# brendisurfs/Distributed-Backtesting-Exploration

Measured on AMD Instinct MI355X. Metric: bar-evals/sec (symbols x params x bars), higher is better.
Workload: dtype f64+int64; 1 GPU; BASELINE config 2: SMA fast/slow crossover, 5,000 symbols x 2,520 daily bars x 400 params per GPU; symbols_total=5000, symbols_per_gpu=5000, bars=2520, params=400, topk=100, parallelism=dp1 (contiguous symbol shards; exchange: none)

## Files before the change

### distributed-backtesting-exploration_amd/csrc/device_common.h

```cpp
#pragma once
#include <type_traits>

#include "internal.h"

namespace bt {

__host__ __device__ inline uint64_t trade_mix(uint64_t w) {
    const uint64_t z = (w ^ (w >> 29)) * 0xBF58476D1CE4E5B9ULL;
    return z ^ (z >> 32);
}
__host__ __device__ inline uint64_t trade_mix_et(uint32_t e, uint32_t t, bool lg) {
    const uint32_t lo = e ^ (t << 2) ^ (t << 31);
    const uint32_t hi = (t >> 1) ^ (lg ? 0x40000002u : 0u);
    const uint64_t z = (((uint64_t)hi << 32) | lo) * 0xBF58476D1CE4E5B9ULL;
    return z ^ (z >> 32);
}
constexpr int kDstLevels = 6;
constexpr int kKeyStride = kTile + 1;

typedef __int128 i128;
typedef __attribute__((address_space(3))) double lds_f64;

struct __attribute__((aligned(16))) Agg {
    int32_t mx, mn, dd, du;
};

__device__ __forceinline__ Agg agg_one(int32_t x) { return Agg{x, x, 0, 0}; }

__device__ __forceinline__ Agg agg_sel(bool c, const Agg& a, const Agg& b) {
    return Agg{c ? a.mx : b.mx, c ? a.mn : b.mn, c ? a.dd : b.dd, c ? a.du : b.du};
}

__device__ __forceinline__ Agg agg_merge(const Agg& a, const Agg& b) {
    Agg r;
    r.mx = max(a.mx, b.mx);
    r.mn = min(a.mn, b.mn);
    r.dd = max(max(a.dd, b.dd), a.mx - b.mn);
    r.du = max(max(a.du, b.du), b.mx - a.mn);
    return r;
}

__device__ __forceinline__ int dst_row(int a, int b) {
    return __builtin_clz((unsigned)(a ^ b) | 1u) - (32 - kDstLevels);
}
__device__ __forceinline__ const Agg* dst_rowp(const Agg* D, int a, int b) {
    return D - (32 - kDstLevels) * kTile + __builtin_clz((unsigned)(a ^ b) | 1u) * kTile;
}

__device__ __forceinline__ Agg dst_query(const Agg* D, const int32_t* cT, int a, int b) {
    if (a == b) return agg_one(cT[a]);
    const int r = dst_row(a, b);
    return agg_merge(D[r * kTile + a], D[r * kTile + b]);
}

__device__ __forceinline__ Agg dst_query_bf(const Agg* D, int a, int b) {
    const Agg* Dr = dst_rowp(D, a, b);
    return agg_merge(Dr[a], Dr[b]);
}

__device__ __forceinline__ Agg dst_query_w(const Agg* D, int a, int b) {
    const Agg* Dr = dst_rowp(D, a, b);
    const int4 u = *reinterpret_cast<const int4*>(Dr + a);
    const int4 v = *reinterpret_cast<const int4*>(Dr + b);
    asm volatile("" ::"v"(u.x), "v"(u.y), "v"(u.z), "v"(u.w), "v"(v.x), "v"(v.y), "v"(v.z), "v"(v.w));
    return agg_merge(Agg{u.x, u.y, u.z, u.w}, Agg{v.x, v.y, v.z, v.w});
}

__host__ __device__ inline double key_recip(int W) { return (1.0 / (double)W) * (1.0 + 0x1p-47); }

constexpr Agg kAggId = {0, 0x7FFFFFFF, 0, 0};

__device__ __forceinline__ int64_t wave_iscan_i64(int64_t x) {
    uint32_t lo = (uint32_t)x, hi = (uint32_t)((uint64_t)x >> 32);
#define BT_DPP_STEP(ctrl, rmask)                                                      \
    {                                                                                 \
        const uint32_t ylo = __builtin_amdgcn_update_dpp(0u, lo, ctrl, rmask, 0xf, false); \
        const uint32_t yhi = __builtin_amdgcn_update_dpp(0u, hi, ctrl, rmask, 0xf, false); \
        const uint64_t r = (((uint64_t)hi << 32) | lo) + (((uint64_t)yhi << 32) | ylo);   \
        lo = (uint32_t)r;                                                             \
        hi = (uint32_t)(r >> 32);                                                     \
    }
    BT_DPP_STEP(0x111, 0xf)
    BT_DPP_STEP(0x112, 0xf)
    BT_DPP_STEP(0x114, 0xf)
    BT_DPP_STEP(0x118, 0xf)
    BT_DPP_STEP(0x142, 0xa)
    BT_DPP_STEP(0x143, 0xc)
#undef BT_DPP_STEP
    return (int64_t)(((uint64_t)hi << 32) | lo);
}

#define BT_S64_CTRLS(X)                                                                   \
    X("row_shr:1 row_mask:0xf bank_mask:0xf bound_ctrl:1")                                \
    X("row_shr:2 row_mask:0xf bank_mask:0xf bound_ctrl:1")                                \
    X("row_shr:4 row_mask:0xf bank_mask:0xf bound_ctrl:1")                                \
    X("row_shr:8 row_mask:0xf bank_mask:0xf bound_ctrl:1")                                \
    X("row_bcast:15 row_mask:0xa bank_mask:0xf")                                          \
    X("row_bcast:31 row_mask:0xc bank_mask:0xf")
__device__ __forceinline__ int64_t wave_iscan_i64_ac(int64_t x) {
    uint32_t lo = (uint32_t)x, hi = (uint32_t)((uint64_t)x >> 32);
#define BT_S64_ONE(ctrl)                                                                   \
    "s_nop 1\n"                                                                            \
    "v_add_co_u32_dpp %0, vcc, %0, %0 " ctrl "\n"                                          \
    "v_addc_co_u32_dpp %1, vcc, %1, %1, vcc " ctrl "\n"
    asm volatile(BT_S64_CTRLS(BT_S64_ONE) "s_nop 1" : "+v"(lo), "+v"(hi) : : "vcc");
#undef BT_S64_ONE
    return (int64_t)(((uint64_t)hi << 32) | lo);
}
__device__ __forceinline__ void wave_iscan2_i64_ac(int64_t& x, int64_t& y) {
    uint32_t xl = (uint32_t)x, xh = (uint32_t)((uint64_t)x >> 32);
    uint32_t yl = (uint32_t)y, yh = (uint32_t)((uint64_t)y >> 32);
#define BT_S64_TWO(ctrl)                                                                   \
    "v_add_co_u32_dpp %0, vcc, %0, %0 " ctrl "\n"                                          \
    "v_addc_co_u32_dpp %1, vcc, %1, %1, vcc " ctrl "\n"                                    \
    "v_add_co_u32_dpp %2, vcc, %2, %2 " ctrl "\n"                                          \
    "v_addc_co_u32_dpp %3, vcc, %3, %3, vcc " ctrl "\n"
    asm volatile("s_nop 1\n" BT_S64_CTRLS(BT_S64_TWO) "s_nop 1"
                 : "+v"(xl), "+v"(xh), "+v"(yl), "+v"(yh) : : "vcc");
#undef BT_S64_TWO
    x = (int64_t)(((uint64_t)xh << 32) | xl);
    y = (int64_t)(((uint64_t)yh << 32) | yl);
// ... 98 lines not shown
```

### distributed-backtesting-exploration_amd/csrc/engine.cpp

```cpp
#include <hip/hip_runtime.h>

#include <algorithm>
#include <atomic>
#include <charconv>
#include <chrono>
#include <cmath>
#include <cstdio>
#include <cstdlib>
#include <cstring>
#include <exception>
#include <string>
#include <thread>
#include <unordered_map>
#include <vector>

#include "csv.h"
#include "internal.h"

using namespace bt;

namespace {

thread_local std::string g_err;

void set_err(const std::string& s) { g_err = s; }

struct HipFail {
    std::string msg;
};

#define HIPCHK(x)                                                                              \
    do {                                                                                       \
        hipError_t e_ = (x);                                                                   \
        if (e_ != hipSuccess)                                                                  \
            throw HipFail{std::string(#x) + ": " + hipGetErrorString(e_)};                     \
    } while (0)

template <class T>
struct DevBuf {
    T* p = nullptr;
    size_t n = 0;
    void ensure(size_t want) {
        if (want <= n && p) return;
        if (p) (void)hipFree(p);
        p = nullptr;
        n = 0;
        if (want == 0) return;
        HIPCHK(hipMalloc(&p, want * sizeof(T)));
        n = want;
    }
    void release() {
        if (p) (void)hipFree(p);
        p = nullptr;
        n = 0;
    }
};

uint32_t next_pow2(uint32_t x) {
    uint32_t r = 1;
    while (r < x) r <<= 1;
    return r;
}

}

void bt::set_last_error(const std::string& s) { set_err(s); }

constexpr int64_t kNtrRing = 64;

struct bt_engine {
    bt_config cfg{};
    std::vector<int32_t> ax[4];
    Grid grid{};
    int32_t P = 0;
    hipStream_t stream = nullptr;
    bool own_stream = false;
    DevBuf<int32_t> d_axes[4];
    std::vector<SymDesc> syms;
    int64_t rows = 0;
    DevBuf<SymDesc> d_syms;
    DevBuf<int32_t> d_c, d_h, d_l;
    DevBuf<bt_summary> d_sum[2];
    DevBuf<uint64_t> d_key[2];
    DevBuf<unsigned long long> d_ntr_ring;
    unsigned long long* ntr[2] = {nullptr, nullptr};
    int cur = 0;
    int64_t nrun = 0;
    DevBuf<bt_sums> d_sums;
    DevBuf<bt_trade> d_trades;
    int32_t seg_req = 0, seg_burn = kDefaultBurnTiles, seg_last = 1;
    bool seg_burn_set = false;
    DevBuf<SegRec> d_seg;
    DevBuf<double> d_segema;
    DevBuf<unsigned long long> d_refixed;
    DevBuf<unsigned long long> d_dbg;
    hipStream_t tstream = nullptr;
    hipEvent_t ev_kdone = nullptr;
    hipEvent_t ev_tdone[2] = {nullptr, nullptr};
    bool tdone_armed[2] = {false, false};
    DevBuf<unsigned int> d_hist, d_counts;
    DevBuf<unsigned long long> d_state, d_above, d_cand;
    DevBuf<bt_topk_rec> d_top;
    bt_topk_rec* h_top = nullptr;
    bt_topk_rec* h_slot[BT_PIPE_SLOTS] = {};
    hipEvent_t slot_ev[BT_PIPE_SLOTS] = {};
    bool slot_armed[BT_PIPE_SLOTS] = {};
    bool topk_ready = false;
    bool ran = false;
    std::vector<std::pair<hipEvent_t, hipEvent_t>> ev_pending, ev_pool;
    double kernel_ms = 0.0;
    int64_t launches = 0;
    int32_t* h_stage[3] = {nullptr, nullptr, nullptr};
    size_t stage_rows[3] = {0, 0, 0};
    bt_summary* h_sum = nullptr;
    size_t h_sum_n = 0;
    hipEvent_t ev_batch[4] = {nullptr, nullptr, nullptr, nullptr};
    bt_batch_profile prof{};
    int64_t n_errors = 0;
    DevBuf<uint8_t> d_replay;
};

namespace {

void activate(bt_engine* e) { HIPCHK(hipSetDevice(e->cfg.device)); }

bool has_hl(const bt_engine* e) { return e->cfg.strategy == BT_BOLL; }

const char* kernel_name(int32_t strategy) {
    switch (strategy) {
        case BT_SMA_CROSS: return "bt::sma_kernel";
// ... 39 lines not shown
            e->grid.nc = e->grid.nd = 1;
            e->grid.band_bps = c.band_bps;
            e->grid.wmax = *std::max_element(e->ax[1].begin(), e->ax[1].end());
            e->grid.ring = (e->grid.wmax + 5 * kTile - 1) / kTile * kTile;
            if (ema_lds_bytes(e->grid, 1) > 160 * 1024) return "EMA grid needs more LDS than a CU has (OLS windows too long)";
            break;
        }
        case BT_BOLL: {
            if (!(err = copy_axis(0, c.bwin, c.n_bwin, "bwin", 1, 1 << 16)).empty()) return err;
            if (!(err = copy_axis(1, c.k_num, c.n_k, "k_num", 0, 1 << 20)).empty()) return err;
            if (!(err = copy_axis(2, c.sl_bps, c.n_sl, "sl_bps", 0, 9999)).empty()) return err;
            if (!(err = copy_axis(3, c.tp_bps, c.n_tp, "tp_bps", 0, 9999)).empty()) return err;
            if (c.k_den < 1 || c.k_den > (1 << 20)) return "k_den out of range";
            e->grid.na = c.n_bwin;
            e->grid.nb = c.n_k;
            e->grid.nc = c.n_sl;
            e->grid.nd = c.n_tp;
            e->grid.k_den = c.k_den;
            e->grid.wmax = *std::max_element(e->ax[0].begin(), e->ax[0].end());
            const int64_t kmax = std::max<int64_t>(c.k_den, *std::max_element(e->ax[1].begin(), e->ax[1].end()));
            if ((int64_t)e->grid.wmax * kmax >= (1LL << 32)) return "Bollinger grid outside the exact int128 range (window * k >= 2^32)";
            e->grid.ring = (e->grid.wmax + 4 * kTile - 1) / kTile * kTile;
            for (int q = 0; q < 8; ++q) {
                const int64_t kn = q < c.n_k ? e->ax[1][q] : 0;
                e->grid.kn2[q] = (double)(kn * kn);
            }
            e->grid.kmin_idx = (int32_t)(std::min_element(e->ax[1].begin(), e->ax[1].end()) - e->ax[1].begin());
            if (boll_lds_bytes(e->grid) > 160 * 1024) return "Bollinger grid needs more LDS than a CU has (windows too long)";
            break;
        }
        default:
            return "unknown strategy";
    }
    const int64_t P = (int64_t)e->grid.na * e->grid.nb * e->grid.nc * e->grid.nd;
    if (P <= 0 || P > (1 << 20)) return "parameter grid too large";
    e->P = (int32_t)P;
    e->grid.n_params = e->P;
    if (c.annualization <= 0) return "annualization must be positive";
    e->grid.sqrt_ann = std::sqrt((double)c.annualization);
    if (c.topk < 0 || c.topk > kTopkMax) return "topk must be in [0, 1024]";
    if ((c.flags & BT_FLAG_PARITY) && c.trade_cap <= 0) return "parity mode needs trade_cap > 0";
    return "";
}

void upload_grid(bt_engine* e) {
    const int32_t** dst[4] = {&e->grid.a, &e->grid.b, &e->grid.c, &e->grid.d};
    for (int i = 0; i < 4; ++i) {
        *dst[i] = nullptr;
        if (e->ax[i].empty()) continue;
        e->d_axes[i].ensure(e->ax[i].size());
        HIPCHK(hipMemcpy(e->d_axes[i].p, e->ax[i].data(), e->ax[i].size() * 4, hipMemcpyHostToDevice));
        *dst[i] = e->d_axes[i].p;
    }
}

int64_t align_rows(int64_t bars) { return (bars + kRowAlign - 1) / kRowAlign * kRowAlign; }

void sync_all(bt_engine* e);

void set_dataset(bt_engine* e, std::vector<SymDesc>&& syms, int64_t rows) {
    sync_all(e);
    e->syms = std::move(syms);
    e->rows = rows;
    const size_t n_sym = e->syms.size();
    e->d_syms.ensure(std::max<size_t>(1, n_sym));
    if (n_sym)
        HIPCHK(hipMemcpyAsync(e->d_syms.p, e->syms.data(), n_sym * sizeof(SymDesc),
                              hipMemcpyHostToDevice, e->stream));
    const size_t r = std::max<int64_t>(1, rows);
    e->d_c.ensure(r);
    if (has_hl(e)) {
        e->d_h.ensure(r);
        e->d_l.ensure(r);
    }
    e->ran = false;
}

void layout(bt_engine* e, int32_t n_sym, const int32_t* bars, const int64_t* ids) {
    std::vector<SymDesc> syms((size_t)n_sym);
    int64_t off = 0;
    for (int32_t s = 0; s < n_sym; ++s) {
        syms[s].off = off;
        syms[s].bars = bars[s];
        syms[s].id = (int32_t)ids[s];
        off += align_rows(bars[s]);
    }
    set_dataset(e, std::move(syms), off);
}

template <class T>
void ensure_pinned(T*& p, size_t& have, size_t want) {
    if (want <= have && p) return;
    if (p) HIPCHK(hipHostFree(p));
    p = nullptr;
    have = 0;
    HIPCHK(hipHostMalloc(&p, std::max<size_t>(want, 1) * sizeof(T)));
    have = std::max<size_t>(want, 1);
}

TopkWork topk_work(bt_engine* e) {
    return TopkWork{e->d_hist.p, e->d_state.p, e->d_counts.p, e->d_above.p, e->d_cand.p,
                    kTopkCap, e->d_top.p + 1, reinterpret_cast<int32_t*>(e->d_top.p)};
}

void sync_all(bt_engine* e) {
    HIPCHK(hipStreamSynchronize(e->stream));
// ... 540 lines not shown
        e = new bt_engine();
        e->cfg = *cfg;
        std::string m = validate_and_copy(e, *cfg);
        if (!m.empty()) {
            delete e;
            return fail(m);
        }
        e->cfg.fast = e->cfg.slow = e->cfg.span = e->cfg.ols = nullptr;
        e->cfg.bwin = e->cfg.k_num = e->cfg.sl_bps = e->cfg.tp_bps = nullptr;
        int ndev = 0;
        HIPCHK(hipGetDeviceCount(&ndev));
        if (cfg->device < 0 || cfg->device >= ndev)
            throw HipFail{"HIP device " + std::to_string(cfg->device) + " not present (" +
                          std::to_string(ndev) + " visible)"};
        activate(e);
        if (cfg->stream) {
            e->stream = (hipStream_t)cfg->stream;
        } else {
            HIPCHK(hipStreamCreateWithFlags(&e->stream, hipStreamNonBlocking));
            e->own_stream = true;
        }
        HIPCHK(hipStreamCreateWithFlags(&e->tstream, hipStreamNonBlocking));
        HIPCHK(hipEventCreateWithFlags(&e->ev_kdone, hipEventDisableTiming));
        for (int b = 0; b < 2; ++b) HIPCHK(hipEventCreateWithFlags(&e->ev_tdone[b], hipEventDisableTiming));
        upload_grid(e);
#ifdef BT_PROFILING
        if (const char* ab = getenv("BT_ABLATE")) e->grid.ablate = atoi(ab);
#endif
        return e;
    } catch (const HipFail& f) {
        delete e;
        return fail(f.msg);
    } catch (const std::exception& x) {
        delete e;
        return fail(std::string("exception: ") + x.what());
    }
}

void bt_engine_destroy(bt_engine* e) {
    if (!e) return;
    try {
        (void)hipSetDevice(e->cfg.device);
        if (e->stream) (void)hipStreamSynchronize(e->stream);
        if (e->tstream) (void)hipStreamSynchronize(e->tstream);
        for (auto& ev : e->ev_pending) {
            (void)hipEventDestroy(ev.first);
            (void)hipEventDestroy(ev.second);
        }
        for (auto& ev : e->ev_pool) {
            (void)hipEventDestroy(ev.first);
            (void)hipEventDestroy(ev.second);
        }
        for (auto& b : e->d_axes) b.release();
        e->d_syms.release();
        e->d_c.release();
        e->d_h.release();
        e->d_l.release();
        for (int b = 0; b < 2; ++b) {
            e->d_sum[b].release();
            e->d_key[b].release();
            if (e->ev_tdone[b]) (void)hipEventDestroy(e->ev_tdone[b]);
            e->ev_tdone[b] = nullptr;
            e->tdone_armed[b] = false;
        }
        if (e->ev_kdone) (void)hipEventDestroy(e->ev_kdone);
        e->ev_kdone = nullptr;
        e->d_ntr_ring.release();
        e->d_sums.release();
        e->d_trades.release();
        e->d_seg.release();
        e->d_segema.release();
        e->d_refixed.release();
        e->d_dbg.release();
        e->d_replay.release();
        e->d_hist.release();
        e->d_counts.release();
        e->d_state.release();
        e->d_above.release();
        e->d_cand.release();
        e->d_top.release();
        if (e->h_top) (void)hipHostFree(e->h_top);
        e->h_top = nullptr;
        for (int i = 0; i < BT_PIPE_SLOTS; ++i) {
            if (e->h_slot[i]) (void)hipHostFree(e->h_slot[i]);
            if (e->slot_ev[i]) (void)hipEventDestroy(e->slot_ev[i]);
            e->h_slot[i] = nullptr;
            e->slot_ev[i] = nullptr;
            e->slot_armed[i] = false;
        }
        e->topk_ready = false;
        for (int i = 0; i < 3; ++i)
            if (e->h_stage[i]) (void)hipHostFree(e->h_stage[i]);
        if (e->h_sum) (void)hipHostFree(e->h_sum);
        for (hipEvent_t& ev : e->ev_batch)
            if (ev) (void)hipEventDestroy(ev);
        if (e->own_stream && e->stream) (void)hipStreamDestroy(e->stream);
        if (e->tstream) (void)hipStreamDestroy(e->tstream);
        e->tstream = nullptr;
    } catch (...) {
    }
    delete e;
}

int32_t bt_num_params(const bt_engine* e) { return e ? e->P : -1; }

int32_t bt_set_segments(bt_engine* e, int32_t segments, int32_t burn_tiles) {
// ... 350 lines not shown
```

### distributed-backtesting-exploration_amd/csrc/internal.h

```cpp
#pragma once
#include <hip/hip_runtime.h>
#include <stdint.h>

#include <string>

#include "../../include/bt.h"

#ifdef BT_PROFILING
#define BT_ABL(g, bit) (((g).ablate & (bit)) != 0)
#define BT_PRIO(g, shift, dflt) (BT_ABL(g, 1 << 20) ? (((g).ablate >> (shift)) & 3) : (dflt))
#else
#define BT_ABL(g, bit) false
#define BT_PRIO(g, shift, dflt) (dflt)
#endif
constexpr int kDbgSlots = 80, kDbgBlocks = 1024;

namespace bt {

constexpr int kTile = 64;
constexpr int kRowAlign = 64;

struct SymDesc {
    int64_t off;
    int32_t bars;
    int32_t id;
};

struct Grid {
    int32_t strategy;
    int32_t n_params;
    int32_t na, nb, nc, nd;
    int32_t band_bps, k_den;
    int32_t wmax;
    int32_t ring;
    double sqrt_ann;
    double kn2[8];
    int32_t kmin_idx;
    int32_t ablate;
    const int32_t* a;
    const int32_t* b;
    const int32_t* c;
    const int32_t* d;
};

struct Out {
    bt_summary* sum;
    uint64_t* key;
    bt_sums* sums;
    bt_trade* trades;
    int32_t trade_cap;
    unsigned long long* n_trades;
    unsigned long long* dbg;
};

struct SegRec {
    int32_t ntr, expo;
    int32_t start_pos, start_e;
    int32_t end_pos, end_e, end_ce, pad;
    int32_t end_agg[4];
    int64_t R;
    int64_t A, B, C, D;
    uint64_t h;
    uint64_t s1lo;
    int64_t s1hi;
    uint64_t s2lo;
    int64_t s2hi;
};
static_assert(sizeof(SegRec) == 128, "SegRec layout");
struct SmaSegRec {
    int32_t ntr;
    int32_t e0;
    int32_t start_pos, end_pos;
    int32_t end_e, end_ce;
    int32_t x1, px1;
    int32_t agg1[4];
    int32_t end_agg[4];
    int64_t R;
    int64_t B, C, D;
    uint64_t h;
    uint64_t s1lo, s2lo;
    int32_t s1hi, s2hi;
};
static_assert(sizeof(SmaSegRec) == sizeof(SegRec), "SmaSegRec is one 128-B SegRec slot");
struct SegArgs {
    SegRec* rec;
    int8_t* pos;
    unsigned long long* refixed;
    double* ema;
    int32_t G;
    int32_t burn_tiles;
};
constexpr int kDefaultBurnTiles = 64;
constexpr int kEmaSegStride = 128;
hipError_t launch_gen(const SymDesc* syms, int32_t n_sym, uint64_t seed, int32_t freq,
                      int32_t* o, int32_t* h, int32_t* l, int32_t* c, hipStream_t st);
size_t sma_lds_bytes(const Grid& g);
// ... 14 lines not shown
size_t boll_lds_bytes(const Grid& g);
hipError_t launch_ema_ols(const SymDesc* syms, int32_t n_sym, const int32_t* close, const Grid& g,
                          const Out& out, bool parity, const SegArgs& seg, hipStream_t st);
int32_t ema_auto_segments(int32_t n_sym, int32_t n_params, int32_t max_bars, int32_t burn_tiles);
int32_t ema_burn_tiles(int32_t max_span);
hipError_t launch_boll(const SymDesc* syms, int32_t n_sym, const int32_t* high, const int32_t* low,
                       const int32_t* close, const Grid& g, const Out& out, bool parity,
                       const SegArgs& seg, hipStream_t st);
int32_t boll_auto_segments(int32_t n_sym, int32_t n_params, int32_t max_bars);

struct ReplayLane {
    int64_t off;
    int32_t bars;
    int32_t param;
};
struct ReplayOut {
    bt_summary* sum;
    bt_trade* trades;
    int32_t trade_cap;
    int64_t* equity;
    int8_t* pos;
    int64_t pitch;
};
hipError_t launch_replay(const ReplayLane* lanes, int32_t n, const int32_t* high, const int32_t* low,
                         const int32_t* close, const Grid& g, const ReplayOut& o, hipStream_t st);

constexpr int kTopkCap = 2048;
constexpr int kTopkMax = 1024;
struct TopkWork {
    unsigned int* hist;
    unsigned long long* state;
    unsigned int* counts;
    unsigned long long* above;
    unsigned long long* cand;
    int cap;
    bt_topk_rec* out;
    int32_t* out_n;
};
hipError_t launch_topk(const uint64_t* key, const bt_summary* sum, const SymDesc* syms,
                       int64_t n, int32_t P, int32_t k, const TopkWork& w, hipStream_t st, bool lds_free_hist = false);
hipError_t launch_topk_init(const TopkWork& w, hipStream_t st);

void set_last_error(const std::string& s);
inline bool topk_less(const bt_topk_rec& a, const bt_topk_rec& b);
struct ExchangeView {
    hipStream_t tstream;
    int32_t device, topk;
    const bt_topk_rec* d_top;
    const unsigned long long* d_ntr;
    int64_t bar_evals;
};
bool engine_exchange_view(bt_engine* e, ExchangeView& v, std::string& err);
void engine_exchange_enqueued(bt_engine* e);

__host__ __device__ inline uint64_t order_key(double x) {
    union { double d; uint64_t u; } v;
    v.d = x;
    return (v.u >> 63) ? ~v.u : (v.u | 0x8000000000000000ULL);
}

__host__ __device__ inline double i128_to_double(uint64_t lo, int64_t hi) {
    const bool neg = hi < 0;
    uint64_t mh = (uint64_t)hi, ml = lo;
    if (neg) {
        ml = ~ml + 1;
        mh = ~mh + (ml == 0 ? 1 : 0);
    }
    if (mh == 0 && ml == 0) return 0.0;
    int lz = mh ? __builtin_clzll(mh) : 64 + __builtin_clzll(ml);
    uint64_t nh, nl;
    if (lz >= 64) {
        nh = ml << (lz - 64);
        nl = 0;
    } else if (lz == 0) {
        nh = mh;
        nl = ml;
    } else {
        nh = (mh << lz) | (ml >> (64 - lz));
        nl = ml << lz;
    }
    uint64_t mant = nh >> 11;
    const uint64_t rem_hi = nh & 0x7FFULL;
    const uint64_t half = 0x400ULL;
    bool up;
    if (rem_hi > half) up = true;
    else if (rem_hi < half) up = false;
    else up = (nl != 0) || (mant & 1);
    mant += up ? 1 : 0;
    double r = (double)mant;
#ifdef __HIP_DEVICE_COMPILE__
    r = ldexp(r, 75 - lz);
#else
    r = __builtin_ldexp(r, 75 - lz);
#endif
    return neg ? -r : r;
}

inline bool topk_less(const bt_topk_rec& a, const bt_topk_rec& b) {
    const uint64_t ka = order_key(a.sharpe), kb = order_key(b.sharpe);
    if (ka != kb) return ka > kb;
    if (a.sym != b.sym) return a.sym < b.sym;
    return a.param < b.param;
}

__host__ __device__ inline double sharpe_fx(uint64_t s1lo, int64_t s1hi, uint64_t s2lo,
                                            int64_t s2hi, int32_t bars, double sqrt_ann) {
// ... 10 lines not shown
```

### distributed-backtesting-exploration_amd/csrc/k_sma.hip

```cpp
#include <algorithm>
#include <cmath>
#include <cstdlib>

#include "tile_common.h"

namespace bt {

namespace {

constexpr int kKS = kTile + 4;
constexpr int kStages = 3;
constexpr int kDstStages = 2;
constexpr int kKeyGrab = 4;
constexpr int kCmpDepth1 = 2;

struct SmaLds {
    size_t ring, keys, invw, win, dst, ct, ql, nar, ctr, total;
};

__host__ __device__ inline SmaLds sma_lds_layout(int ring, int nw) {
    SmaLds L;
    size_t o = 0;
    auto take = [&](size_t bytes) { size_t r = o; o += (bytes + 15) & ~size_t(15); return r; };
    L.ring = take((size_t)ring * 8);
    const int nwp = (nw + kKeyGrab - 1) / kKeyGrab * kKeyGrab;
    L.keys = take((size_t)2 * nwp * kKS * 4);
    L.invw = take((size_t)nwp * 8);
    L.win = take((size_t)nwp * 4);
    L.dst = take((size_t)kDstStages * kDstLevels * kTile * sizeof(Agg));
    L.ct = take((size_t)kStages * kTile * 4);
    L.ql = take((size_t)kStages * 2 * kTile * 8);
    L.nar = take((size_t)kStages * 4);
    L.ctr = take(4);
    L.total = o;
    return L;
}

struct ScanCarry {
    int64_t P;
    int32_t prevc;
    uint32_t tv;
};

__device__ __forceinline__ int32_t load_close(const int32_t* __restrict__ crow, int B, int t) {
    return t < B ? crow[t] : 0;
}

__device__ __forceinline__ void stage_ring(int32_t c, int B, int t0, int lane, int R, double* ring,
                                           int32_t* cT, int64_t* ql, int32_t* narrow,
                                           ScanCarry& cy) {
    const int t = t0 + lane;
    const bool valid = t < B;
    const int32_t cp = (int32_t)__builtin_amdgcn_update_dpp((uint32_t)cy.prevc, (uint32_t)c,
                                                            0x138, 0xf, 0xf, false);
    const int64_t inc = wave_iscan_i64((int64_t)c);
    ring[(t + 1) & (R - 1)] = (double)(cy.P + inc);
    cT[lane] = c;
    int64_t q = 0, q2 = 0;
    uint32_t dv = 0;
    if (valid && t >= 1) {
        fixed_ret(c, cp, q, q2);
        dv = (uint32_t)abs(c - cp);
    }
    ql[lane] = wave_iscan_i64(q);
    ql[kTile + lane] = wave_iscan_i64(q2);
    const bool big = __ballot(dv >= (1u << 25)) != 0;
    const uint32_t tvt = __builtin_amdgcn_readlane(wave_iscan_u32(min(dv, 1u << 25)), 63);
    cy.tv = big ? (1u << 31) : min(cy.tv + tvt, 1u << 31);
    if (lane == 0) *narrow = cy.tv < (1u << 30);
    cy.P += lane63_i64(inc);
    cy.prevc = (int32_t)__builtin_amdgcn_readlane((uint32_t)c, 63);
}

__device__ __forceinline__ uint32_t grab_issue(uint32_t* ctr, int lane) {
    uint32_t v = 0;
    if (lane == 0) v = atomicAdd(ctr, (uint32_t)kKeyGrab);
    return v;
}

__device__ __forceinline__ int32_t floor_key(double F, double iw) {
    return (int32_t)(F * iw);
}

__host__ __device__ inline uint32_t key_round_len(int nwp, int nwaves) {
    return (uint32_t)kKeyGrab * ((uint32_t)nwp / kKeyGrab + 1 + (uint32_t)nwaves);
}

__device__ __forceinline__ void stage_keys(int t0, int B, int nw, int nwp, int nf, int wmax, int R,
                                           double* ring, const int32_t* win,
                                           const double* invw, int32_t* K, uint32_t* ctr,
                                           uint32_t round, int nwaves, int lane,
                                           const int32_t* cTr, Agg* Dr) {
    const int t = t0 + lane;
    const double top = ring[(t + 1) & (R - 1)];
    const bool full = t0 + 1 - wmax >= 0 && t0 + kTile <= B;
    const uint32_t base = round * key_round_len(nwp, nwaves);
    uint32_t w = __builtin_amdgcn_readlane(grab_issue(ctr, lane), 0) - base;
#pragma unroll 1
    while (w < (uint32_t)(nwp + kKeyGrab)) {
        const uint32_t vn = grab_issue(ctr, lane);
        if (w == 0) {
            dst_build<true>(cTr[lane], lane, Dr);
            w = __builtin_amdgcn_readlane(vn, 0) - base;
            continue;
        }
        w -= kKeyGrab;
        int Wv[kKeyGrab];
        double Iv[kKeyGrab], Fv[kKeyGrab];
#pragma unroll
        for (int q = 0; q < kKeyGrab; q += 4) {
            const int4 W4 = *reinterpret_cast<const int4*>(win + w + q);
            Wv[q] = W4.x; Wv[q + 1] = W4.y; Wv[q + 2] = W4.z; Wv[q + 3] = W4.w;
        }
#pragma unroll
        for (int q = 0; q < kKeyGrab; q += 2) {
            const double2 I2 = *reinterpret_cast<const double2*>(invw + w + q);
            Iv[q] = I2.x; Iv[q + 1] = I2.y;
        }
#pragma unroll
        for (int q = 0; q < kKeyGrab; ++q) {
            Wv[q] = __builtin_amdgcn_readfirstlane(Wv[q]);
            Fv[q] = top - ring[(t + 1 - Wv[q]) & (R - 1)];
        }
        int32_t* Kw = K + w * kKS + lane;
        if (full) {
#pragma unroll
            for (int q = 0; q < kKeyGrab; ++q) Kw[q * kKS] = floor_key(Fv[q], Iv[q]);
        } else {
            const bool tin = t < B;
#pragma unroll
            for (int q = 0; q < kKeyGrab; ++q) {
                const int32_t kq = floor_key(Fv[q], Iv[q]);
                Kw[q * kKS] = (tin && t + 1 - Wv[q] >= 0) ? kq : ((int)(w + q) < nf ? -1 : -2);
            }
        }
        w = __builtin_amdgcn_readlane(vn, 0) - base;
    }
}

__device__ __forceinline__ void cmp4(uint32_t& l, uint32_t& z, const int4& x, const int4& y) {
    const uint32_t d0 = (uint32_t)(x.x - y.x), d1 = (uint32_t)(x.y - y.y);
    const uint32_t d2 = (uint32_t)(x.z - y.z), d3 = (uint32_t)(x.w - y.w);
    l = __builtin_amdgcn_alignbit(l, d0, 31);
    l = __builtin_amdgcn_alignbit(l, d1, 31);
    l = __builtin_amdgcn_alignbit(l, d2, 31);
    l = __builtin_amdgcn_alignbit(l, d3, 31);
    z = min(min(z, d0), d1);
    z = min(min(z, d2), d3);
}

__device__ __forceinline__ uint64_t eq_word(const int32_t* k1, const int32_t* k2) {
    uint64_t e = 0;
#pragma unroll 1
    for (int b = 0; b < kTile; ++b) e |= (uint64_t)(k1[b] == k2[b]) << b;
    return e;
}

}

struct SmaAcct {
    int32_t pos, e, ce, sb, ntr, e0;
    int32_t g32, m32, r32;
    int64_t R, gap, mdd;
    uint64_t ps1, ps2, h;
    I96 s1, s2;
    Agg agg;
    int64_t Bq, C, D;
    int32_t carried, x1, px1;
    Agg agg1;
};


template <bool PARITY, bool MERGE = true, bool SEG = false, bool NARROW = false>
__device__ __forceinline__ void sma_close(SmaAcct& a, const Agg& seg, int t, int32_t cx,
                                          bt_trade* tr, int cap) {
    const Agg st = MERGE ? agg_merge(a.agg, seg) : seg;
    if (SEG && MERGE && a.carried) {
        a.x1 = t;
        a.px1 = cx;
        a.agg1 = st;
        a.carried = 0;
        a.ntr++;
        return;
    }
    const bool lg = a.pos > 0;
    const int32_t lo = lg ? st.mn - a.ce : a.ce - st.mx;
    const int32_t hi = lg ? st.mx - a.ce : a.ce - st.mn;
    const int32_t path = lg ? st.dd : st.du;
    const int32_t pnl = lg ? cx - a.ce : a.ce - cx;
// ... 55 lines not shown
                     "v"((uint32_t)(qb >> 32)));
        seg = agg_merge(d1, d2);
    } else {
        seg = dst_query_bf(D, a.sb, b);
        cx = cT[b];
        qb = (uint64_t)ql[b];
    }
    alt = qb - alt;
    sma_close<PARITY, FIRST, SEG, NARROW>(a, seg, t0 + b, cx, tr, cap);
    sma_open<FIRST>(a, b, t0 + b, cx, -a.pos);
}

template <bool PARITY, bool ONE_TRIP, bool SEG, bool NARROW>
__device__ __forceinline__ void sma_flips(SmaAcct& a, uint64_t F, int t0, int bl, uint64_t LONG,
                                          const int32_t* cT, const int64_t* ql, const Agg* D,
                                          bt_trade* tr, int cap) {
    const uint64_t FX = (bl >= 0 && bl < 64) ? (F & (1ULL << bl)) : 0ULL;
    F ^= FX;
    if (a.pos == 0 && F != 0) {
        const int b = __builtin_ctzll(F);
        F &= F - 1;
        const int np = ((LONG >> b) & 1) ? 1 : -1;
        const uint64_t qx = (uint64_t)ql[b];
        a.ps1 += np > 0 ? (uint64_t)0 - qx : qx;
        a.ps2 -= (uint64_t)ql[kTile + b];
        a.e0 = t0 + b;
        sma_open(a, b, t0 + b, cT[b], np);
    }
    uint64_t alt = 0;
    if (F) sma_reverse<PARITY, ONE_TRIP, true, SEG, NARROW>(a, F, alt, t0, cT, ql, D, tr, cap);
    while (F) sma_reverse<PARITY, ONE_TRIP, false, SEG, NARROW>(a, F, alt, t0, cT, ql, D, tr, cap);
    a.ps1 += a.pos > 0 ? (uint64_t)0 - (alt << 1) : alt << 1;
    if (FX) {
        const int b = bl;
        const uint64_t qx = (uint64_t)ql[b];
        sma_close<PARITY, true, SEG, NARROW>(a, dst_query_bf(D, a.sb, b), t0 + b, cT[b], tr, cap);
        a.ps1 += a.pos > 0 ? qx : (uint64_t)0 - qx;
        a.ps2 += (uint64_t)ql[kTile + b];
        a.pos = 0;
    }
}

template <bool PARITY, bool STAMPS, bool ONE_TRIP, bool SEG>
__device__ __forceinline__ void sma_body(const SymDesc* __restrict__ syms,
                                         const int32_t* __restrict__ close, const Grid& g,
                                         const Out& out, int dedicated, const SegArgs& sg,
                                         int fix_seg) {
    extern __shared__ __attribute__((aligned(16))) unsigned char smem[];
    const int nf = g.na, ns = g.nb, nw = nf + ns;
    const int R = g.ring;
    const SmaLds LL = sma_lds_layout(R, nw);
    double* ring = reinterpret_cast<double*>(smem + LL.ring);
    int32_t* keys = reinterpret_cast<int32_t*>(smem + LL.keys);
    double* invw = reinterpret_cast<double*>(smem + LL.invw);
    int32_t* win = reinterpret_cast<int32_t*>(smem + LL.win);
    Agg* dst = reinterpret_cast<Agg*>(smem + LL.dst);
    int32_t* cts = reinterpret_cast<int32_t*>(smem + LL.ct);
    int64_t* qls = reinterpret_cast<int64_t*>(smem + LL.ql);
    int32_t* nars = reinterpret_cast<int32_t*>(smem + LL.nar);
    uint32_t* ctr = reinterpret_cast<uint32_t*>(smem + LL.ctr);

    const int tid = threadIdx.x;
    const int lane = tid & 63;
    const int wave = __builtin_amdgcn_readfirstlane(tid >> 6);
    const int nwaves = (int)blockDim.x >> 6;
    const bool helper = (tid >> 6) == nwaves - 1;
    const int nparam_threads = dedicated ? (int)blockDim.x - 64 : (int)blockDim.x;
    const SymDesc sd = syms[blockIdx.x];
    const int B = sd.bars;
    const int ntiles = (B + kTile - 1) / kTile;
    const int P = g.n_params;
    const int j = blockIdx.y * nparam_threads + tid;
    const bool active = tid < nparam_threads && j < P;
    const int kf = active ? j % nf : 0;
    const int ks = nf + (active ? j / nf : 0);
    const int p = (kf * ns) + (ks - nf);
    const int32_t* crow = close + sd.off;

    SegRange sr{0, 0, 0, 0, ntiles};
    SmaSegRec* mine = nullptr;
    size_t ipos = 0, npos = 0;
    if (SEG) {
        sr = seg_range(sg, fix_seg, ntiles, g.wmax);
        const size_t per_seg = (size_t)gridDim.x * P;
        ipos = sr.seg * per_seg + (size_t)blockIdx.x * P + p;
        npos = (size_t)sg.G * per_seg;
        mine = reinterpret_cast<SmaSegRec*>(sg.rec) + ipos;
        if (fix_seg > 0) {
            if (!__syncthreads_or(active && sg.pos[ipos] != sg.pos[npos + ipos - per_seg])) return;
            if (tid == 0) atomicAdd(sg.refixed, 1ULL);
        }
    }
    const int T_scan = sr.T_scan, T_walk = sr.T_walk, T_acct = sr.T_acct, T_end = sr.T_end;

    const int nwp = (nw + kKeyGrab - 1) / kKeyGrab * kKeyGrab;
    const uint32_t key_round = key_round_len(nwp, nwaves);
    for (int w = tid; w < nwp; w += blockDim.x) {
        const int W = w < nf ? g.a[w] : (w < nw ? g.b[w - nf] : 1);
        win[w] = W;
        invw[w] = key_recip(W);
    }
    if (tid == 0) {
        ring[(T_scan * kTile) & (R - 1)] = 0.0;
        *ctr = (uint32_t)T_walk * key_round;
    }
    __syncthreads();
    const int warm = max(win[kf], win[ks]) - 1;
    const uint32_t fsw = (uint32_t)win[kf] | ((uint32_t)win[ks] << 16);

    ScanCarry cy{0, (T_scan > 0 && T_scan * kTile - 1 < B) ? crow[T_scan * kTile - 1] : 0};
    if (SEG && helper && T_scan < T_walk) {
        constexpr int kLookAhead = 8;
        int32_t cn[kLookAhead];
#pragma unroll
        for (int u = 0; u < kLookAhead; ++u) cn[u] = load_close(crow, B, (T_scan + u) * kTile + lane);
#pragma unroll 1
        for (int T0 = T_scan; T0 < T_walk; T0 += kLookAhead) {
#pragma unroll
            for (int u = 0; u < kLookAhead; ++u) {
                const int T = T0 + u;
                if (T < T_walk) {
                    const int32_t c = cn[u];
                    cn[u] = load_close(crow, B, (T + kLookAhead) * kTile + lane);
                    const int64_t inc = wave_iscan_i64((int64_t)c);
                    ring[(T * kTile + lane + 1) & (R - 1)] = (double)(cy.P + inc);
                    cy.P += lane63_i64(inc);
                    cy.prevc = (int32_t)__builtin_amdgcn_readlane((uint32_t)c, 63);
                }
            }
        }
    }
    int32_t cpre = 0;
    if (helper) {
        const int b0 = T_walk * kTile;
        const int32_t c0 = load_close(crow, B, b0 + lane), c1 = load_close(crow, B, b0 + kTile + lane);
        cpre = load_close(crow, B, b0 + 2 * kTile + lane);
        const int s0 = T_walk % kStages, s1 = (T_walk + 1) % kStages;
        if (T_walk < T_end) stage_ring(c0, B, b0, lane, R, ring, cts + s0 * kTile, qls + s0 * 2 * kTile, nars + s0, cy);
        __syncthreads();
        if (T_walk + 1 < T_end)
            stage_ring(c1, B, b0 + kTile, lane, R, ring, cts + s1 * kTile, qls + s1 * 2 * kTile, nars + s1, cy);
    } else {
        __syncthreads();
    }
    if (T_walk < T_end)
        stage_keys(T_walk * kTile, B, nw, nwp, nf, g.wmax, R, ring, win, invw,
                   keys + (T_walk & 1) * nwp * kKS, ctr, (uint32_t)T_walk, nwaves, lane,
                   cts + (T_walk % kStages) * kTile, dst + (T_walk % kDstStages) * kDstLevels * kTile);
    __syncthreads();

    SmaAcct a;
    a.pos = a.e = a.ce = a.sb = a.ntr = a.e0 = 0;
    a.g32 = a.m32 = a.r32 = 0;
    a.R = a.gap = a.mdd = 0;
    a.ps1 = a.ps2 = 0;
    a.h = 0;
    a.s1.clear();
    a.s2.clear();
    a.agg = kAggId;
    a.Bq = a.C = a.D = kNegInf;
    a.carried = a.x1 = a.px1 = 0;
    a.agg1 = kAggId;
    int32_t start_pos = 0;
    if (SEG && fix_seg > 0 && active) a.pos = sg.pos[npos + ipos - (size_t)gridDim.x * P];
    auto enter_acct = [&]() {
        start_pos = a.pos;
        a.carried = a.pos != 0;
        a.agg = kAggId;
        a.sb = 0;
        a.R = 0;
        a.Bq = a.C = a.D = kNegInf;
        a.ntr = 0;
        a.h = 0;
        a.s1.clear();
        a.s2.clear();
        a.ps1 = a.ps2 = 0;
        a.e0 = -1;
        a.x1 = -1;
        a.px1 = 0;
        a.agg1 = kAggId;
    };
    if (SEG && T_walk == T_acct) enter_acct();
    bt_trade* tr = nullptr;
    auto result_index = [&]() -> size_t {
        int le = lane;
        asm volatile("" : "+v"(le));
        const int je = blockIdx.y * nparam_threads + wave * 64 + le;
        return (size_t)blockIdx.x * P + (size_t)((je % nf) * ns + je / nf);
    };
    const size_t gi = (size_t)blockIdx.x * P + p;
    if (PARITY && active) tr = out.trades + gi * out.trade_cap;
    const int cap = out.trade_cap;

    constexpr bool stamps = STAMPS;
    uint64_t st_acc[7] = {0, 0, 0, 0, 0, 0, 0};
    uint64_t st_prev = 0;
#define BT_STAMP(i)                                             \
    if (stamps) {                                               \
        const uint64_t now_ = __builtin_amdgcn_s_memtime();     \
        st_acc[i] += now_ - st_prev;                            \
        st_prev = now_;                                         \
    }
    if (stamps) st_prev = __builtin_amdgcn_s_memtime();

    auto tile_step = [&](auto narrow_tag, const int k) __attribute__((always_inline)) {
        constexpr bool NARROW = decltype(narrow_tag)::value;
        const int t0 = k * kTile;
        if (helper && k + 2 < T_end && !BT_ABL(g, 1)) {
            if (!BT_ABL(g, 32)) __builtin_amdgcn_s_setprio(2);
            const int s = (k + 2) % kStages;
            stage_ring(cpre, B, t0 + 2 * kTile, lane, R, ring, cts + s * kTile,
                       qls + s * 2 * kTile, nars + s, cy);
            cpre = load_close(crow, B, t0 + 3 * kTile + lane);
            __builtin_amdgcn_s_setprio(0);
        }
        BT_STAMP(0)
        if (SEG && active && k == T_acct && k != T_walk) enter_acct();
        if (active) {
            if (ONE_TRIP) __builtin_amdgcn_s_setprio(1);
            const int s = k % kStages;
            const int32_t* cT = cts + s * kTile;
            const int64_t* ql = qls + s * 2 * kTile;
            const Agg* D = dst + (k % kDstStages) * kDstLevels * kTile;
            const int32_t* K = keys + (k & 1) * nwp * kKS;
            const int4* k1 = reinterpret_cast<const int4*>(K + kf * kKS);
            const int4* k2 = reinterpret_cast<const int4*>(K + ks * kKS);
            uint32_t l0 = 0, l1 = 0, z = ~0u;
            if (!BT_ABL(g, 4)) {
#pragma unroll
                for (int v = 0; v < 16; ++v) {
                    if (v < 8) cmp4(l0, z, k1[v], k2[v]);
                    else cmp4(l1, z, k1[v], k2[v]);
                    if (ONE_TRIP ? ((v % kCmpDepth1) == kCmpDepth1 - 1) : (v & 1))
                        __builtin_amdgcn_sched_barrier(0);
                }
            }
            BT_STAMP(2)
            uint64_t L = ((uint64_t)__builtin_bitreverse32(l1) << 32) | __builtin_bitreverse32(l0);
            const int lastdec = B - 2 - t0;
            const int wb = warm - t0;
            const int bl = B - 1 - t0;
            uint64_t LONG, F;
            if (z != 0 && wb <= 0 && lastdec >= 63) {
                LONG = ~L;
                F = (LONG ^ ((LONG << 1) | (uint64_t)(a.pos == 1))) | (uint64_t)(a.pos == 0);
            } else {
                uint64_t vm = lastdec >= 63 ? ~0ULL : (lastdec < 0 ? 0ULL : ((1ULL << (lastdec + 1)) - 1));
                vm &= wb <= 0 ? ~0ULL : (wb >= 64 ? 0ULL : (~0ULL << wb));
                uint64_t G, T = 0;
                if (z != 0) {
                    G = ~L & vm;
                } else {
                    const uint64_t E = eq_word(K + kf * kKS, K + ks * kKS);
                    G = ~(L | E) & vm;
                    T = E & vm;
                }
                L &= vm;
                while (T) {
                    const int b = __builtin_ctzll(T);
                    T &= T - 1;
                    const int t = t0 + b;
                    const double top = ring[(t + 1) & (R - 1)];
                    const int fw = (int)(fsw & 0xffffu), sw = (int)(fsw >> 16);
                    const int64_t Fs = (int64_t)(top - ring[(t + 1 - fw) & (R - 1)]) * sw;
                    const int64_t Lf = (int64_t)(top - ring[(t + 1 - sw) & (R - 1)]) * fw;
                    G |= (uint64_t)(Fs > Lf) << b;
                    L |= (uint64_t)(Fs < Lf) << b;
                }
                uint64_t SHORT;
                {
                    const uint64_t A = ~L;
                    const uint64_t s1 = A + G;
                    uint64_t cout = s1 < A;
                    const uint64_t sum = s1 + (uint64_t)(a.pos == 1);
                    cout |= sum < s1;
                    LONG = ((sum ^ A ^ G) >> 1) | (cout << 63);
                }
                {
                    const uint64_t A = ~G;
                    const uint64_t s1 = A + L;
                    uint64_t cout = s1 < A;
                    const uint64_t sum = s1 + (uint64_t)(a.pos == -1);
                    cout |= sum < s1;
                    SHORT = ((sum ^ A ^ L) >> 1) | (cout << 63);
                }
                if (bl < 64) {
                    const uint64_t keep = bl <= 0 ? 0ULL : ((1ULL << bl) - 1);
                    LONG &= keep;
                    SHORT &= keep;
                }
                const uint64_t pL = (LONG << 1) | (uint64_t)(a.pos == 1);
                const uint64_t pS = (SHORT << 1) | (uint64_t)(a.pos == -1);
                F = (LONG ^ pL) | (SHORT ^ pS);
            }
            BT_STAMP(3)
            uint64_t Fw = F;
            if (BT_ABL(g, 8)) {
                asm volatile("" ::"v"((uint32_t)Fw), "v"((uint32_t)(Fw >> 32)));
                Fw = 0;
            }
            sma_flips<PARITY, ONE_TRIP, SEG, NARROW>(a, Fw, t0, bl, LONG, cT, ql, D, tr, cap);
            BT_STAMP(4)
            if (a.pos != 0) {
                a.agg = agg_merge(a.agg, dst_query_bf(D, a.sb, kTile - 1));
                a.sb = 0;
                const uint64_t q63 = (uint64_t)ql[kTile - 1];
                a.ps1 += a.pos > 0 ? q63 : (uint64_t)0 - q63;
                a.ps2 += (uint64_t)ql[2 * kTile - 1];
            }
            if ((k & 1) || k + 1 == T_end) {
                a.s1.add((int64_t)a.ps1);
                a.s2.add((int64_t)a.ps2);
                a.ps1 = a.ps2 = 0;
            }
            BT_STAMP(5)
            if (ONE_TRIP) __builtin_amdgcn_s_setprio(0);
        }
        if (k + 1 < T_end && !BT_ABL(g, 2))
            stage_keys(t0 + kTile, B, nw, nwp, nf, g.wmax, R, ring, win, invw, keys + ((k + 1) & 1) * nwp * kKS,
                       ctr, (uint32_t)(k + 1), nwaves, lane, cts + ((k + 1) % kStages) * kTile,
                       dst + ((k + 1) % kDstStages) * kDstLevels * kTile);
        BT_STAMP(1)
        __syncthreads();
        BT_STAMP(6)
    };
    int k = T_walk;
    if (!SEG && k < T_end) {
        bool nar = __builtin_amdgcn_readfirstlane(nars[k % kStages]) != 0;
        while (nar) {
            const int32_t nn = k + 1 < T_end ? nars[(k + 1) % kStages] : 0;
            tile_step(std::true_type{}, k);
            nar = __builtin_amdgcn_readfirstlane(nn) != 0;
            ++k;
        }
        a.gap = (uint32_t)a.g32;
        a.mdd = (uint32_t)a.m32;
        a.R = a.r32;
    }
    for (; k < T_end; ++k) tile_step(std::false_type{}, k);
#undef BT_STAMP
    if (stamps && lane == 0) {
        unsigned long long* d = out.dbg + (helper ? 8 : 0);
        for (int i = 0; i < 7; ++i) atomicAdd(&d[i], (unsigned long long)st_acc[i]);
        atomicAdd(&d[7], 1ULL);
    }
    if (SEG) {
        if (active) {
            SmaSegRec r;
            r.ntr = a.ntr;
            r.e0 = a.e0;
            r.start_pos = start_pos;
            r.end_pos = a.pos;
            r.end_e = a.carried ? -1 : a.e;
            r.end_ce = a.ce;
            r.x1 = a.x1;
            r.px1 = a.px1;
            const Agg g1 = a.x1 >= 0 ? a.agg1 : a.agg;
            r.agg1[0] = g1.mx;
            r.agg1[1] = g1.mn;
            r.agg1[2] = g1.dd;
            r.agg1[3] = g1.du;
            r.end_agg[0] = a.agg.mx;
            r.end_agg[1] = a.agg.mn;
            r.end_agg[2] = a.agg.dd;
            r.end_agg[3] = a.agg.du;
            r.R = a.R;
            r.B = a.Bq;
            r.C = a.C;
            r.D = a.D;
            r.h = a.h;
            r.s1lo = a.s1.lo;
            r.s1hi = a.s1.hi;
// ... 204 lines not shown
```

Baseline: 4522 billion bar-evals/s.

## Load SMA window keys via scalar constant loads and mirror ring for contiguous reads

Moves the per-window lengths and reciprocals out of LDS into a host-precomputed global table that is read through constant address space (scalar loads), freeing LDS and removing the per-block init loop. Adds a mirrored tail to the LDS close-sum ring so per-lane reads use a lane-offset base pointer. Also skips the per-tile signal walk for tiles before the smallest warmup window in the wave. The mirror write conditions and the early-skip add complexity and may be a correctness risk at wrap boundaries.

```diff
diff --git a/distributed-backtesting-exploration_amd/csrc/device_common.h b/distributed-backtesting-exploration_amd/csrc/device_common.h
--- a/distributed-backtesting-exploration_amd/csrc/device_common.h
+++ b/distributed-backtesting-exploration_amd/csrc/device_common.h
@@ -65,8 +65,6 @@
     asm volatile("" ::"v"(u.x), "v"(u.y), "v"(u.z), "v"(u.w), "v"(v.x), "v"(v.y), "v"(v.z), "v"(v.w));
     return agg_merge(Agg{u.x, u.y, u.z, u.w}, Agg{v.x, v.y, v.z, v.w});
 }
-
-__host__ __device__ inline double key_recip(int W) { return (1.0 / (double)W) * (1.0 + 0x1p-47); }
 
 constexpr Agg kAggId = {0, 0x7FFFFFFF, 0, 0};
 
diff --git a/distributed-backtesting-exploration_amd/csrc/engine.cpp b/distributed-backtesting-exploration_amd/csrc/engine.cpp
--- a/distributed-backtesting-exploration_amd/csrc/engine.cpp
+++ b/distributed-backtesting-exploration_amd/csrc/engine.cpp
@@ -76,6 +76,8 @@
     hipStream_t stream = nullptr;
     bool own_stream = false;
     DevBuf<int32_t> d_axes[4];
+    DevBuf<int32_t> d_kwin;
+    DevBuf<double> d_krecip;
     std::vector<SymDesc> syms;
     int64_t rows = 0;
     DevBuf<SymDesc> d_syms;
@@ -221,6 +223,21 @@
         HIPCHK(hipMemcpy(e->d_axes[i].p, e->ax[i].data(), e->ax[i].size() * 4, hipMemcpyHostToDevice));
         *dst[i] = e->d_axes[i].p;
     }
+    e->grid.kwin = nullptr;
+    e->grid.krecip = nullptr;
+    if (e->cfg.strategy == BT_SMA_CROSS) {
+        std::vector<int32_t> win(e->ax[0]);
+        win.insert(win.end(), e->ax[1].begin(), e->ax[1].end());
+        win.resize((win.size() + kKeyGrab - 1) / kKeyGrab * kKeyGrab, 1);
+        std::vector<double> recip(win.size());
+        for (size_t i = 0; i < win.size(); ++i) recip[i] = key_recip(win[i]);
+        e->d_kwin.ensure(win.size());
+        e->d_krecip.ensure(win.size());
+        HIPCHK(hipMemcpy(e->d_kwin.p, win.data(), win.size() * sizeof(int32_t), hipMemcpyHostToDevice));
+        HIPCHK(hipMemcpy(e->d_krecip.p, recip.data(), recip.size() * sizeof(double), hipMemcpyHostToDevice));
+        e->grid.kwin = e->d_kwin.p;
+        e->grid.krecip = e->d_krecip.p;
+    }
 }
 
 int64_t align_rows(int64_t bars) { return (bars + kRowAlign - 1) / kRowAlign * kRowAlign; }
@@ -867,6 +884,8 @@
             (void)hipEventDestroy(ev.second);
         }
         for (auto& b : e->d_axes) b.release();
+        e->d_kwin.release();
+        e->d_krecip.release();
         e->d_syms.release();
         e->d_c.release();
         e->d_h.release();
diff --git a/distributed-backtesting-exploration_amd/csrc/internal.h b/distributed-backtesting-exploration_amd/csrc/internal.h
--- a/distributed-backtesting-exploration_amd/csrc/internal.h
+++ b/distributed-backtesting-exploration_amd/csrc/internal.h
@@ -41,7 +41,10 @@
     const int32_t* b;
     const int32_t* c;
     const int32_t* d;
-};
+    const int32_t* kwin;
+    const double* krecip;
+};
+constexpr int kKeyGrab = 4;
 
 struct Out {
     bt_summary* sum;
@@ -162,6 +165,8 @@
 };
 bool engine_exchange_view(bt_engine* e, ExchangeView& v, std::string& err);
 void engine_exchange_enqueued(bt_engine* e);
+
+__host__ __device__ inline double key_recip(int W) { return (1.0 / (double)W) * (1.0 + 0x1p-47); }
 
 __host__ __device__ inline uint64_t order_key(double x) {
     union { double d; uint64_t u; } v;
diff --git a/distributed-backtesting-exploration_amd/csrc/k_sma.hip b/distributed-backtesting-exploration_amd/csrc/k_sma.hip
--- a/distributed-backtesting-exploration_amd/csrc/k_sma.hip
+++ b/distributed-backtesting-exploration_amd/csrc/k_sma.hip
@@ -11,22 +11,20 @@
 constexpr int kKS = kTile + 4;
 constexpr int kStages = 3;
 constexpr int kDstStages = 2;
-constexpr int kKeyGrab = 4;
+constexpr int kRingMirror = kTile;
 constexpr int kCmpDepth1 = 2;
 
 struct SmaLds {
-    size_t ring, keys, invw, win, dst, ct, ql, nar, ctr, total;
+    size_t ring, keys, dst, ct, ql, nar, ctr, total;
 };
 
 __host__ __device__ inline SmaLds sma_lds_layout(int ring, int nw) {
     SmaLds L;
     size_t o = 0;
     auto take = [&](size_t bytes) { size_t r = o; o += (bytes + 15) & ~size_t(15); return r; };
-    L.ring = take((size_t)ring * 8);
+    L.ring = take((size_t)(ring + kRingMirror) * 8);
     const int nwp = (nw + kKeyGrab - 1) / kKeyGrab * kKeyGrab;
     L.keys = take((size_t)2 * nwp * kKS * 4);
-    L.invw = take((size_t)nwp * 8);
-    L.win = take((size_t)nwp * 4);
     L.dst = take((size_t)kDstStages * kDstLevels * kTile * sizeof(Agg));
     L.ct = take((size_t)kStages * kTile * 4);
     L.ql = take((size_t)kStages * 2 * kTile * 8);
@@ -44,6 +42,15 @@
 
 __device__ __forceinline__ int32_t load_close(const int32_t* __restrict__ crow, int B, int t) {
     return t < B ? crow[t] : 0;
+}
+
+__device__ __forceinline__ void ring_store(double* ring, int R, int t0, int lane, double v) {
+    const int i = (t0 + lane + 1) & (R - 1);
+    ring[i] = v;
+    const int rb = t0 & (R - 1);
+    if (rb == 0 || rb == R - kTile) {
+        if (i < kRingMirror) ring[R + i] = v;
+    }
 }
 
 __device__ __forceinline__ void stage_ring(int32_t c, int B, int t0, int lane, int R, double* ring,
@@ -54,7 +61,7 @@
     const int32_t cp = (int32_t)__builtin_amdgcn_update_dpp((uint32_t)cy.prevc, (uint32_t)c,
                                                             0x138, 0xf, 0xf, false);
     const int64_t inc = wave_iscan_i64((int64_t)c);
-    ring[(t + 1) & (R - 1)] = (double)(cy.P + inc);
+    ring_store(ring, R, t0, lane, (double)(cy.P + inc));
     cT[lane] = c;
     int64_t q = 0, q2 = 0;
     uint32_t dv = 0;
@@ -86,55 +93,66 @@
     return (uint32_t)kKeyGrab * ((uint32_t)nwp / kKeyGrab + 1 + (uint32_t)nwaves);
 }
 
-__device__ __forceinline__ void stage_keys(int t0, int B, int nw, int nwp, int nf, int wmax, int R,
-                                           double* ring, const int32_t* win,
-                                           const double* invw, int32_t* K, uint32_t* ctr,
-                                           uint32_t round, int nwaves, int lane,
+struct KeyGroup {
+    int32_t W[kKeyGrab];
+    double I[kKeyGrab];
+};
+typedef __attribute__((address_space(4))) const int32_t const_i32;
+typedef __attribute__((address_space(4))) const double const_f64;
+__device__ __forceinline__ KeyGroup key_group(const int32_t* kwin, const double* krecip,
+                                              uint32_t w, int nwp) {
+    const uint32_t i = min(w - (uint32_t)kKeyGrab, (uint32_t)(nwp - kKeyGrab));
+    const_i32* cw = (const_i32*)kwin + i;
+    const_f64* cr = (const_f64*)krecip + i;
+    KeyGroup g;
+#pragma unroll
+    for (int q = 0; q < kKeyGrab; ++q) {
+        g.W[q] = cw[q];
+        g.I[q] = cr[q];
+    }
+    return g;
+}
+
+__device__ __forceinline__ void stage_keys(int t0, int B, int nwp, int nf, int wmax, int R,
+                                           const double* ring, const int32_t* __restrict__ kwin,
+                                           const double* __restrict__ krecip, int32_t* K,
+                                           uint32_t* ctr, uint32_t round, int nwaves, int lane,
                                            const int32_t* cTr, Agg* Dr) {
     const int t = t0 + lane;
-    const double top = ring[(t + 1) & (R - 1)];
+    const double* ringl = ring + lane;
+    const double top = ringl[(t0 + 1) & (R - 1)];
     const bool full = t0 + 1 - wmax >= 0 && t0 + kTile <= B;
     const uint32_t base = round * key_round_len(nwp, nwaves);
     uint32_t w = __builtin_amdgcn_readlane(grab_issue(ctr, lane), 0) - base;
+    KeyGroup gw = key_group(kwin, krecip, w, nwp);
 #pragma unroll 1
     while (w < (uint32_t)(nwp + kKeyGrab)) {
         const uint32_t vn = grab_issue(ctr, lane);
         if (w == 0) {
             dst_build<true>(cTr[lane], lane, Dr);
             w = __builtin_amdgcn_readlane(vn, 0) - base;
+            gw = key_group(kwin, krecip, w, nwp);
             continue;
         }
         w -= kKeyGrab;
-        int Wv[kKeyGrab];
-        double Iv[kKeyGrab], Fv[kKeyGrab];
-#pragma unroll
-        for (int q = 0; q < kKeyGrab; q += 4) {
-            const int4 W4 = *reinterpret_cast<const int4*>(win + w + q);
-            Wv[q] = W4.x; Wv[q + 1] = W4.y; Wv[q + 2] = W4.z; Wv[q + 3] = W4.w;
-        }
-#pragma unroll
-        for (int q = 0; q < kKeyGrab; q += 2) {
-            const double2 I2 = *reinterpret_cast<const double2*>(invw + w + q);
-            Iv[q] = I2.x; Iv[q + 1] = I2.y;
-        }
+        int32_t kq[kKeyGrab];
 #pragma unroll
         for (int q = 0; q < kKeyGrab; ++q) {
-            Wv[q] = __builtin_amdgcn_readfirstlane(Wv[q]);
-            Fv[q] = top - ring[(t + 1 - Wv[q]) & (R - 1)];
+            const double F = top - ringl[(t0 + 1 - gw.W[q]) & (R - 1)];
+            kq[q] = floor_key(F, gw.I[q]);
         }
         int32_t* Kw = K + w * kKS + lane;
         if (full) {
 #pragma unroll
-            for (int q = 0; q < kKeyGrab; ++q) Kw[q * kKS] = floor_key(Fv[q], Iv[q]);
+            for (int q = 0; q < kKeyGrab; ++q) Kw[q * kKS] = kq[q];
         } else {
             const bool tin = t < B;
 #pragma unroll
-            for (int q = 0; q < kKeyGrab; ++q) {
-                const int32_t kq = floor_key(Fv[q], Iv[q]);
-                Kw[q * kKS] = (tin && t + 1 - Wv[q] >= 0) ? kq : ((int)(w + q) < nf ? -1 : -2);
-            }
+            for (int q = 0; q < kKeyGrab; ++q)
+                Kw[q * kKS] = (tin && t + 1 - gw.W[q] >= 0) ? kq[q] : ((int)(w + q) < nf ? -1 : -2);
         }
         w = __builtin_amdgcn_readlane(vn, 0) - base;
+        gw = key_group(kwin, krecip, w, nwp);
     }
 }
 
@@ -296,8 +314,6 @@
     const SmaLds LL = sma_lds_layout(R, nw);
     double* ring = reinterpret_cast<double*>(smem + LL.ring);
     int32_t* keys = reinterpret_cast<int32_t*>(smem + LL.keys);
-    double* invw = reinterpret_cast<double*>(smem + LL.invw);
-    int32_t* win = reinterpret_cast<int32_t*>(smem + LL.win);
     Agg* dst = reinterpret_cast<Agg*>(smem + LL.dst);
     int32_t* cts = reinterpret_cast<int32_t*>(smem + LL.ct);
     int64_t* qls = reinterpret_cast<int64_t*>(smem + LL.ql);
@@ -339,18 +355,20 @@
 
     const int nwp = (nw + kKeyGrab - 1) / kKeyGrab * kKeyGrab;
     const uint32_t key_round = key_round_len(nwp, nwaves);
-    for (int w = tid; w < nwp; w += blockDim.x) {
-        const int W = w < nf ? g.a[w] : (w < nw ? g.b[w - nf] : 1);
-        win[w] = W;
-        invw[w] = key_recip(W);
-    }
     if (tid == 0) {
-        ring[(T_scan * kTile) & (R - 1)] = 0.0;
+        const int i0 = (T_scan * kTile) & (R - 1);
+        ring[i0] = 0.0;
+        if (i0 == 0) ring[R] = 0.0;
         *ctr = (uint32_t)T_walk * key_round;
     }
     __syncthreads();
-    const int warm = max(win[kf], win[ks]) - 1;
-    const uint32_t fsw = (uint32_t)win[kf] | ((uint32_t)win[ks] << 16);
+    const int32_t wf = g.kwin[kf], ws = g.kwin[ks];
+    const int warm = max(wf, ws) - 1;
+    const uint32_t fsw = (uint32_t)wf | ((uint32_t)ws << 16);
+    int wmin = active ? warm : 0x7fffffff;
+#pragma unroll
+    for (int o = 32; o > 0; o >>= 1) wmin = min(wmin, __shfl_xor(wmin, o));
+    const int kfirst = __builtin_amdgcn_readfirstlane(wmin) >> 6;
 
     ScanCarry cy{0, (T_scan > 0 && T_scan * kTile - 1 < B) ? crow[T_scan * kTile - 1] : 0};
     if (SEG && helper && T_scan < T_walk) {
@@ -373,6 +391,7 @@
                 }
             }
         }
+        ring[R + lane] = ring[lane];
     }
     int32_t cpre = 0;
     if (helper) {
@@ -388,7 +407,7 @@
         __syncthreads();
     }
     if (T_walk < T_end)
-        stage_keys(T_walk * kTile, B, nw, nwp, nf, g.wmax, R, ring, win, invw,
+        stage_keys(T_walk * kTile, B, nwp, nf, g.wmax, R, ring, g.kwin, g.krecip,
                    keys + (T_walk & 1) * nwp * kKS, ctr, (uint32_t)T_walk, nwaves, lane,
                    cts + (T_walk % kStages) * kTile, dst + (T_walk % kDstStages) * kDstLevels * kTile);
     __syncthreads();
@@ -460,7 +479,7 @@
         }
         BT_STAMP(0)
         if (SEG && active && k == T_acct && k != T_walk) enter_acct();
-        if (active) {
+        if (active && k >= kfirst) {
             if (ONE_TRIP) __builtin_amdgcn_s_setprio(1);
             const int s = k % kStages;
             const int32_t* cT = cts + s * kTile;
@@ -561,7 +580,7 @@
             if (ONE_TRIP) __builtin_amdgcn_s_setprio(0);
         }
         if (k + 1 < T_end && !BT_ABL(g, 2))
-            stage_keys(t0 + kTile, B, nw, nwp, nf, g.wmax, R, ring, win, invw, keys + ((k + 1) & 1) * nwp * kKS,
+            stage_keys(t0 + kTile, B, nwp, nf, g.wmax, R, ring, g.kwin, g.krecip, keys + ((k + 1) & 1) * nwp * kKS,
                        ctr, (uint32_t)(k + 1), nwaves, lane, cts + ((k + 1) % kStages) * kTile,
                        dst + ((k + 1) % kDstStages) * kDstLevels * kTile);
         BT_STAMP(1)
```

Measured after the change: 4631 billion bar-evals/s (median of 6 runs). +2.4%, better.
